# phlash/java-sdr

Hardware: AMD Instinct MI355X
Metric: IQ Msamples/s through FFT+FIR+BPSK demod, 2048-pt frames (higher is better)
Workload: dtype f64

## Files before the change

java-sdr_amd/csrc/fft_psd.hip:

```cpp
#include "fft_common.h"
#include <math.h>
#include <stdlib.h>
#include <vector>

namespace jsdr {

constexpr bool tw_direct(int P, int R) { return P * R <= 512; }
constexpr int tw_size(int P, int R) { return P <= 1 ? 0 : (tw_direct(P, R) ? 2 * P * (R - 1) : P); }
constexpr int tw_total(int R0, int R1, int R2, int R3)
{
    return tw_size(R0, R1) + (R2 > 1 ? tw_size(R0 * R1, R2) : 0) + (R3 > 1 ? tw_size(R0 * R1 * R2, R3) : 0);
}

constexpr int ilog2_c(int n) { return n <= 1 ? 0 : 1 + ilog2_c(n / 2); }

template <int R, int P>
__device__ __forceinline__ void apply_twiddles(float2 *v, int k, const float2 *tab)
{
    if constexpr (P > 1) {
        if constexpr (tw_direct(P, R)) {
#pragma unroll
            for (int r = 1; r < R; r++) {
                const float4 t = reinterpret_cast<const float4 *>(tab)[(r - 1) * P + k];
                v[r] = cmul2(v[r], make_float2(t.x, t.y), make_float2(t.z, t.w));
            }
        } else {
            float2 w1 = tab[k];
            float2 w[R], wq[R];
            w[1] = w1;
            wq[1] = cquad(w1);
#pragma unroll
            for (int r = 2; r < R; r++) {
                w[r] = (r & 1) ? cmul2(w[r - 1], w1, wq[1]) : cmul2(w[r / 2], w[r / 2], wq[r / 2]);
                wq[r] = cquad(w[r]);
            }
#pragma unroll
            for (int r = 1; r < R; r++) v[r] = cmul2(v[r], w[r], wq[r]);
        }
    }
}

template <int R, int... Rs>
__device__ __forceinline__ void store_lds(float2 *dst, const float2 *v, int j0, int p, std::integer_sequence<int, Rs...>)
{
    ((dst[lds_pad(j0 + Rs * p)] = v[cx_bitrev(Rs, R)]), ...);
}

template <int IN>
struct RawPoint {
    using type = int;
};
template <>
struct RawPoint<IN_F32> {
    using type = float2;
};
template <int N, int T, int IN, int R>
__device__ __forceinline__ void fft_fetch(const FftArgs &a, long long frame, int tid, typename RawPoint<IN>::type (&w)[R])
{
    constexpr int NB = N / R;
    static_assert(NB == T, "one first-pass butterfly per thread");
    const typename RawPoint<IN>::type *src = reinterpret_cast<const typename RawPoint<IN>::type *>(a.in) +
#ifdef JSDR_X_FFT_SMALLSET
        (frame & 8191) * N;
#else
        frame * N;
#endif
#pragma unroll
    for (int r = 0; r < R; r++) {
#ifdef JSDR_X_FFT_NOLOAD
        if constexpr (IN == IN_I16) w[r] = (tid + r * NB) * 2654435761u + (int)(size_t)src;
        else w[r] = make_float2((float)(tid + r), (float)(size_t)src);
#else
        w[r] = src[tid + r * NB];
#endif
    }
}

template <int N, int T, int IN, int OUT, int R, int P, bool FIRST, bool LAST, class RAW = int>
__device__ __forceinline__ void fft_pass(const FftArgs &a, long long frame, bool active, int tid, float2 *buf,
                                         const float2 *tab, Best &best, const RAW *raw = nullptr)
{
    constexpr int NB = N / R;
    static_assert(NB % T == 0, "butterflies per pass must be a multiple of the threads per frame");
    constexpr int ITERS = NB / T;
    constexpr int GROUP = LAST ? 1 : ITERS;
#pragma unroll
    for (int g0 = 0; g0 < ITERS; g0 += GROUP) {
        float2 v[GROUP][R];
#pragma unroll
        for (int gi = 0; gi < GROUP; gi++) {
            const int b = (g0 + gi) * T + tid;
            if constexpr (FIRST) {
                if (active) {
                    if constexpr (IN == IN_I16) {
                        const RAW *w = raw;
                        if ((a.ic | a.qc) == 0) {
#pragma unroll
                            for (int r = 0; r < R; r++)
                                v[gi][r] = make_float2(i16_to_float_java((int)(short)(w[r] & 0xffff)),
                                                       i16_to_float_java(w[r] >> 16));
                        } else {
#pragma unroll
                            for (int r = 0; r < R; r++) {
                                int si = java_short_add((int)(short)(w[r] & 0xffff), a.ic);
                                int sq = java_short_add(w[r] >> 16, a.qc);
                                v[gi][r] = make_float2(i16_to_float_java(si), i16_to_float_java(sq));
                            }
                        }
                    } else {
#pragma unroll
                        for (int r = 0; r < R; r++) v[gi][r] = raw[r];
                    }
                } else {
#pragma unroll
                    for (int r = 0; r < R; r++) v[gi][r] = make_float2(0.f, 0.f);
                }
            } else {
#pragma unroll
                for (int r = 0; r < R; r++) v[gi][r] = buf[lds_pad(b + r * NB)];
            }
            apply_twiddles<R, P>(v[gi], b & (P - 1), tab);
            dft_reg<R>(v[gi]);
        }
        if constexpr (!FIRST && !LAST) __syncthreads();
#pragma unroll
        for (int gi = 0; gi < GROUP; gi++) {
            const int b = (g0 + gi) * T + tid;
            const int k = b & (P - 1);
            const int j0 = (b - k) * R + k;
            if constexpr (!LAST) {
                store_lds<R>(buf, v[gi], j0, P, std::make_integer_sequence<int, R>{});
            } else if (active) {
                if constexpr (OUT == OUT_SPEC) {
                    float2 *dst = reinterpret_cast<float2 *>(a.out) + frame * N;
#pragma unroll
                    for (int r = 0; r < R; r++) dst[j0 + r * P] = v[gi][cx_bitrev(r, R)];
                } else {
                    constexpr float L2 = 3.0102999566398120f;
                    constexpr float OFF = 3.0102999566398120f * (2.0f - 2.0f * (float)ilog2_c(N));
                    float *dst = a.out + frame * (N + 2);
                    float db[R];
#pragma unroll
                    for (int r = 0; r < R; r++) {
                        float2 x = v[gi][cx_bitrev(r, R)];
                        db[r] = L2 * __log2f(x.x * x.x + x.y * x.y) + OFF;
#ifndef JSDR_X_FFT_NOSTORE
                        dst[j0 + r * P] = db[r];
#endif
                    }
                    float gm = db[0];
#pragma unroll
                    for (int r = 1; r < R; r++) gm = fmaxf(gm, db[r]);
                    int gk = 0x7fffffff;
#pragma unroll
                    for (int r = R - 1; r >= 0; r--) gk = (db[r] == gm) ? j0 + r * P : gk;
                    const bool take = (gm > best.v) | ((gm == best.v) & (gk < best.k));
                    best.v = take ? gm : best.v;
                    best.k = take ? gk : best.k;
                }
            }
        }
    }
    if constexpr (!LAST) __syncthreads();
}

template <int N, int T, int IN, int OUT, int R0, int R1, int R2, int R3>
__device__ __forceinline__ void fft_frame(const FftArgs &a, long long frame, long long next, int tid, float2 *buf,
                                          const float2 *tw_lds, float *red_val, int *red_idx, int frame_in_block,
                                          typename RawPoint<IN>::type (&raw)[R0])
{
    using RAW = typename RawPoint<IN>::type;
    constexpr bool active = true;
    constexpr int NPASS = (R1 == 1) ? 1 : (R2 == 1) ? 2 : (R3 == 1) ? 3 : 4;
    static_assert(NPASS >= 2, "the first pass must not be the last");
    static_assert(R0 * R1 * R2 * R3 == N, "radix plan must multiply to N");
    Best best;
    best.v = -3.402823466e+38f;
    best.k = 0x7fffffff;
    constexpr int O1 = 0, O2 = tw_size(R0, R1), O3 = O2 + tw_size(R0 * R1, R2);
    fft_pass<N, T, IN, OUT, R0, 1, true, false, RAW>(a, frame, active, tid, buf, tw_lds, best, raw);
    auto prefetch = [&] { fft_fetch<N, T, IN, R0>(a, next, tid, raw); };
    if constexpr (NPASS == 2) prefetch();
    fft_pass<N, T, IN, OUT, R1, R0, false, NPASS == 2>(a, frame, active, tid, buf, tw_lds + O1, best);
    if constexpr (NPASS >= 3) {
        if constexpr (NPASS == 3) prefetch();
        fft_pass<N, T, IN, OUT, R2, R0 * R1, false, NPASS == 3>(a, frame, active, tid, buf, tw_lds + O2, best);
    }
    if constexpr (NPASS >= 4) {
        prefetch();
        fft_pass<N, T, IN, OUT, R3, R0 * R1 * R2, false, NPASS == 4>(a, frame, active, tid, buf, tw_lds + O3, best);
    }

    if constexpr (OUT == OUT_PSD) {
        float bestv = best.v;
        int bestk = best.k;
        constexpr int W = (T < 64) ? T : 64;
#pragma unroll
        for (int off = W / 2; off >= 1; off >>= 1) {
            float ov = __shfl_xor(bestv, off, W);
            int ok = __shfl_xor(bestk, off, W);
            const bool take = (ov > bestv) | ((ov == bestv) & (ok < bestk));
            bestv = take ? ov : bestv;
            bestk = take ? ok : bestk;
        }
        if constexpr (T > 64) {
            constexpr int NW = T / 64;
            if ((tid & 63) == 0) {
                red_val[frame_in_block * NW + (tid >> 6)] = bestv;
                red_idx[frame_in_block * NW + (tid >> 6)] = bestk;
            }
            __syncthreads();
            if (tid == 0) {
                for (int w = 1; w < NW; w++) {
                    float ov = red_val[frame_in_block * NW + w];
                    int ok = red_idx[frame_in_block * NW + w];
                    if (ov > bestv || (ov == bestv && ok < bestk)) {
                        bestv = ov;
                        bestk = ok;
                    }
                }
            }
        }
        if (tid == 0 && active) {
            int p = (bestv > -3.402823466e+38f) ? 2 * bestk : -1;
            float m = (p >= 0) ? bestv : -3.402823466e+38f;
            const int datlen = 2 * N;
            if (p >= datlen / 2) p -= datlen;
            int hz = (int)((unsigned)p * (unsigned)a.rate) / datlen;
            float *dst = a.out + frame * (N + 2);
            dst[N] = (float)hz;
            dst[N + 1] = m;
        }
    }
}

template <int N, int T, int FPB, int IN, int OUT, int R0, int R1, int R2, int R3, bool TWG = false>
__global__ __launch_bounds__(T *FPB, (N == 2048 ? 4 : 1)) void k_fft(FftArgs a)
{
    extern __shared__ __align__(16) unsigned char smem[];
    constexpr int FE = lds_frame_elems(N);
    constexpr int TWN = TWG ? 0 : tw_total(R0, R1, R2, R3);
    float2 *tw_own = reinterpret_cast<float2 *>(smem);
    float2 *bufs = tw_own + TWN;
    float *red_val = reinterpret_cast<float *>(bufs + (size_t)FPB * FE);
    int *red_idx = reinterpret_cast<int *>(red_val + FPB * ((T + 63) / 64));
    const float2 *tw_lds = TWG ? a.tw : tw_own;

    const int tid_b = threadIdx.x;
    if constexpr (!TWG) {
        for (int i = tid_b; i < TWN; i += T * FPB) tw_own[i] = a.tw[i];
        __syncthreads();
    }

    const int fib = tid_b / T;
    const int tid = tid_b - fib * T;
    float2 *buf = bufs + (size_t)fib * FE;
    const long long ngroups = (a.nframes + FPB - 1) / FPB;
    auto frame_of = [&](long long g) {
        long long f = g * FPB + fib;
        return f < a.nframes ? f : a.nframes - 1;
    };
    typename RawPoint<IN>::type raw[R0];
    if ((long long)blockIdx.x < ngroups) fft_fetch<N, T, IN, R0>(a, frame_of(blockIdx.x), tid, raw);
    for (long long g = blockIdx.x; g < ngroups; g += gridDim.x) {
        const long long gn = g + gridDim.x;
        fft_frame<N, T, IN, OUT, R0, R1, R2, R3>(a, frame_of(g), frame_of(gn < ngroups ? gn : g), tid, buf, tw_lds, red_val,
                                                 red_idx, fib, raw);
        __syncthreads();
    }
}

template <int N, int FPB, int T, int R0, int R1, int R2, int R3, bool TWG = false>
constexpr size_t fft_lds_bytes()
{
    return sizeof(float2) * ((TWG ? (size_t)0 : (size_t)tw_total(R0, R1, R2, R3)) + (size_t)FPB * lds_frame_elems(N)) +
           (sizeof(float) + sizeof(int)) * FPB * ((T + 63) / 64);
}

struct Launcher {
    void (*launch)(const FftArgs &, int grid, hipStream_t) = nullptr;
    int frames_per_block = 0;
    size_t lds_bytes = 0;
    int block = 0;
    int radix[4] = {1, 1, 1, 1};
};

template <int N, int T, int FPB, int IN, int OUT, int R0, int R1, int R2, int R3, bool TWG = false>
static void launch_impl(const FftArgs &a, int grid, hipStream_t s)
{
    constexpr size_t lds = fft_lds_bytes<N, FPB, T, R0, R1, R2, R3, TWG>();
    hipLaunchKernelGGL((k_fft<N, T, FPB, IN, OUT, R0, R1, R2, R3, TWG>), dim3(grid), dim3(T * FPB), lds, s, a);
}

template <int N, int T, int FPB, int R0, int R1, int R2, int R3, bool TWG = false>
static Launcher make_launcher(int in, int out)
{
    Launcher l;
    l.frames_per_block = FPB;
    l.block = T * FPB;
    l.lds_bytes = fft_lds_bytes<N, FPB, T, R0, R1, R2, R3, TWG>();
    l.radix[0] = R0;
    l.radix[1] = R1;
    l.radix[2] = R2;
    l.radix[3] = R3;
    if (in == IN_I16 && out == OUT_PSD) l.launch = launch_impl<N, T, FPB, IN_I16, OUT_PSD, R0, R1, R2, R3, TWG>;
    if (in == IN_F32 && out == OUT_PSD) l.launch = launch_impl<N, T, FPB, IN_F32, OUT_PSD, R0, R1, R2, R3, TWG>;
    if (in == IN_F32 && out == OUT_SPEC) l.launch = launch_impl<N, T, FPB, IN_F32, OUT_SPEC, R0, R1, R2, R3, TWG>;
    return l;
}

static Launcher pick_launcher(int n, int in, int out)
{
    switch (n) {
        case 64: return make_launcher<64, 8, 32, 8, 8, 1, 1>(in, out);
        case 128: return make_launcher<128, 8, 32, 16, 8, 1, 1>(in, out);
        case 256: return make_launcher<256, 16, 16, 16, 16, 1, 1>(in, out);
        case 512: return make_launcher<512, 64, 4, 8, 8, 8, 1>(in, out);
        case 1024: return make_launcher<1024, 64, 4, 16, 8, 8, 1>(in, out);
        case 2048: return make_launcher<2048, 128, 2, 16, 16, 8, 1>(in, out);
        case 4096: return make_launcher<4096, 256, 1, 16, 16, 16, 1>(in, out);
        case 8192: return make_launcher<8192, 512, 1, 16, 16, 8, 4>(in, out);
        default: return Launcher();
    }
}

}

using namespace jsdr;

struct jsdr_fft {
    int n = 0;
    int rate = 0;
    DevBuf<float2> tw;
    DevBuf<unsigned char> in_stage;
    DevBuf<float> out_stage;
    PinnedStage pin;
    bool pin_lazy_done = false;
    int num_cu = 256;
    bool mixed = false;
    MixedPlan mplan;
    bool rt = false;
    bool direct = false;
    long long last_items = 0, last_grid = 0;
    int share_wgs_per_cu = 0;
};

static int fft_run(jsdr_fft *h, const void *in_dev, int in_kind, int out_kind, long long nframes, int ic, int qc,
                   float *out_dev, hipStream_t s)
{
    JSDR_REQUIRE(h, "fft: null handle");
    JSDR_REQUIRE(in_dev && out_dev, "fft: null buffer");
    JSDR_REQUIRE(nframes >= 0, "fft: negative frame count");
    if (nframes == 0) return JSDR_OK;
    FftArgs a;
    if (h->rt) {
        a.in = in_dev;
        a.out = out_dev;
        a.tw = h->tw.p;
        a.nframes = nframes;
        a.rate = h->rate;
        a.ic = ic;
        a.qc = qc;
        return rt_launch(a, h->n, in_kind, out_kind, h->num_cu, s);
    }
    if (h->direct) {
        a.in = in_dev;
        a.out = out_dev;
        a.tw = nullptr;
        a.nframes = nframes;
        a.rate = h->rate;
        a.ic = ic;
        a.qc = qc;
        return dft_any_launch(a, h->n, in_kind, out_kind, h->num_cu, s);
    }
    if (h->mixed) {
        a.in = in_dev;
        a.out = out_dev;
        a.tw = h->tw.p;
        a.nframes = nframes;
        a.rate = h->rate;
        a.ic = ic;
        a.qc = qc;
        if (h->mplan.split2)
            return mixed_launch_split2(h->mplan, a, in_kind, out_kind, h->num_cu, s);
        static const int mgrid = [] { const char *e = knob("JSDR_MIXED_GRID"); return e ? atoi(e) : 16; }();
        long long cap = (long long)h->num_cu * mgrid;
        return mixed_launch(h->mplan, a, in_kind, out_kind, (int)(nframes < cap ? nframes : cap), s);
    }
    Launcher l = pick_launcher(h->n, in_kind, out_kind);
    JSDR_REQUIRE(l.launch, "fft: no kernel for n=%d in=%d out=%d", h->n, in_kind, out_kind);
    a.in = in_dev;
    a.out = out_dev;
    a.tw = h->tw.p;
    a.nframes = nframes;
    a.rate = h->rate;
    a.ic = ic;
    a.qc = qc;
    long long groups = (nframes + l.frames_per_block - 1) / l.frames_per_block;
    long long per_cu = (long long)(160 * 1024 / l.lds_bytes);
    if (per_cu < 1) per_cu = 1;
    if (per_cu * l.block > 2048) per_cu = 2048 / l.block;
    static const int mult = [] {
        const char *e = knob("JSDR_FFT_GRID_MULT");
        const int v = e ? atoi(e) : 0;
        return v > 0 ? v : 4;
    }();
    long long cap = (long long)h->num_cu * per_cu * mult;
    static const int abs_grid = [] {
        const char *e = knob("JSDR_FFT_GRID_ABS");
        return e ? atoi(e) : 0;
    }();
    if (abs_grid > 0) cap = abs_grid;
    if (h->share_wgs_per_cu > 0) cap = (long long)h->num_cu * h->share_wgs_per_cu;
    int grid = (int)(groups < cap ? groups : cap);
    h->last_items = groups;
    h->last_grid = grid;
    l.launch(a, grid, s);
    JSDR_LAUNCH_CHECK();
    return JSDR_OK;
}

extern "C" {

int jsdr_fft_create(jsdr_fft **out, int n, int rate)
{
    JSDR_REQUIRE(out, "jsdr_fft_create: null handle pointer");
    *out = nullptr;
    MixedPlan mp;
    const bool pow2 = n >= 64 && n <= 8192 && (n & (n - 1)) == 0;
    const bool mixed = !pow2 && mixed_plan(n, mp);
    const bool rt = !pow2 && !mixed && rt_supported(n);
    const bool direct = !pow2 && !mixed && !rt && dft_any_supported(n);
    JSDR_REQUIRE(pow2 || mixed || rt || direct,
                 "jsdr_fft_create: n=%d unsupported (2 .. 20000 samples)", n);
    JSDR_REQUIRE(rate > 0, "jsdr_fft_create: rate must be positive");
    int dev = 0;
    JSDR_HIP_TRY(hipGetDevice(&dev));
    hipDeviceProp_t prop;
    JSDR_HIP_TRY(hipGetDeviceProperties(&prop, dev));
    jsdr_fft *h = new jsdr_fft();
    h->n = n;
    h->rate = rate;
    h->num_cu = prop.multiProcessorCount > 0 ? prop.multiProcessorCount : 256;
    if (direct) {
        h->direct = true;
        if (h->in_stage.alloc((size_t)n * 8) != JSDR_OK || h->out_stage.alloc((size_t)n + 2) != JSDR_OK) {
            jsdr_fft_destroy(h);
            return JSDR_ERR;
        }
        *out = h;
        return JSDR_OK;
    }
    if (rt) {
        h->rt = true;
        std::vector<float2> rtw;
        rt_twiddles(n, rtw);
        if (h->tw.alloc(rtw.size() ? rtw.size() : 1) != JSDR_OK || h->in_stage.alloc((size_t)n * 8) != JSDR_OK ||
            h->out_stage.alloc((size_t)n + 2) != JSDR_OK ||
            (rtw.size() && hipMemcpy(h->tw.p, rtw.data(), sizeof(float2) * rtw.size(), hipMemcpyHostToDevice) != hipSuccess)) {
            set_error("jsdr_fft_create: run-time-plan setup failed");
            jsdr_fft_destroy(h);
            return JSDR_ERR;
        }
        *out = h;
        return JSDR_OK;
    }
    if (mixed) {
        h->mixed = true;
        h->mplan = mp;
        std::vector<float2> mtw((size_t)mp.tw_count);
        mixed_twiddles(mp, mtw.data());
        if (h->tw.alloc(mtw.size()) != JSDR_OK || h->in_stage.alloc((size_t)n * 8) != JSDR_OK ||
            h->out_stage.alloc((size_t)n + 2) != JSDR_OK ||
            hipMemcpy(h->tw.p, mtw.data(), sizeof(float2) * mtw.size(), hipMemcpyHostToDevice) != hipSuccess) {
            set_error("jsdr_fft_create: mixed-radix setup failed");
            jsdr_fft_destroy(h);
            return JSDR_ERR;
        }
        *out = h;
        return JSDR_OK;
    }
    Launcher l = pick_launcher(n, IN_I16, OUT_PSD);
    std::vector<float2> tw;
    int P = l.radix[0];
    for (int pass = 1; pass < 4 && l.radix[pass] > 1; pass++) {
        const int R = l.radix[pass];
        const double base = -2.0 * 3.14159265358979323846 / ((double)P * (double)R);
        if (tw_direct(P, R)) {
            for (int r = 1; r < R; r++)
                for (int k = 0; k < P; k++) {
                    double ang = base * (double)k * (double)r;
                    const float2 w = make_float2((float)cos(ang), (float)sin(ang));
                    tw.push_back(w);
                    tw.push_back(make_float2(-w.y, w.x));
                }
        } else {
            for (int k = 0; k < P; k++) {
                double ang = base * (double)k;
                tw.push_back(make_float2((float)cos(ang), (float)sin(ang)));
            }
        }
        P *= R;
    }
    if ((int)tw.size() != tw_total(l.radix[0], l.radix[1], l.radix[2], l.radix[3])) {
        set_error("jsdr_fft_create: internal twiddle layout mismatch (%d)", (int)tw.size());
        delete h;
        return JSDR_ERR;
    }
    if (h->tw.alloc(tw.size()) != JSDR_OK || h->in_stage.alloc((size_t)n * 8) != JSDR_OK ||
        h->out_stage.alloc((size_t)n + 2) != JSDR_OK) {
        jsdr_fft_destroy(h);
        return JSDR_ERR;
    }
    if (hipMemcpy(h->tw.p, tw.data(), sizeof(float2) * tw.size(), hipMemcpyHostToDevice) != hipSuccess) {
        set_error("jsdr_fft_create: twiddle upload failed");
        jsdr_fft_destroy(h);
        return JSDR_ERR;
    }
    *out = h;
    return JSDR_OK;
}

int jsdr_fft_destroy(jsdr_fft *h)
{
    if (!h) return JSDR_OK;
    h->tw.release();
    h->in_stage.release();
    h->out_stage.release();
    h->pin.release();
    delete h;
    return JSDR_OK;
}

int jsdr_fft_batch_f32(jsdr_fft *h, const float *iq_dev, int64_t nframes, float *psd_dev, void *stream)
{
    return fft_run(h, iq_dev, IN_F32, OUT_PSD, nframes, 0, 0, psd_dev, as_stream(stream));
}

int jsdr_fft_set_cu_share(jsdr_fft *h, int wgs_per_cu)
{
    JSDR_REQUIRE(h && wgs_per_cu >= 0 && wgs_per_cu <= 16, "jsdr_fft_set_cu_share: bad argument");
    h->share_wgs_per_cu = wgs_per_cu;
    return JSDR_OK;
}

const char *jsdr_fft_kernel(jsdr_fft *h)
{
    if (!h) return "";
    return h->rt ? "k_fft_rt" : h->direct ? "k_dft_any" : h->mixed ? (h->mplan.split2 ? "k_fft_mixed_dual" : "k_fft_mixed") : "k_fft";
}

int jsdr_fft_last_launch(jsdr_fft *h, int64_t *work_items, int64_t *workgroups)
{
    JSDR_REQUIRE(h && work_items && workgroups, "jsdr_fft_last_launch: null argument");
    *work_items = h->last_items;
    *workgroups = h->last_grid;
    return JSDR_OK;
}

int jsdr_fft_batch_i16(jsdr_fft *h, const int16_t *raw_dev, int64_t nframes, int ic, int qc, float *psd_dev,
                       void *stream)
{
    return fft_run(h, raw_dev, IN_I16, OUT_PSD, nframes, ic, qc, psd_dev, as_stream(stream));
}

int jsdr_fft_spectrum_f32(jsdr_fft *h, const float *iq_dev, int64_t nframes, float *spec_dev, void *stream)
{
    return fft_run(h, iq_dev, IN_F32, OUT_SPEC, nframes, 0, 0, spec_dev, as_stream(stream));
}

static int fft_receive(jsdr_fft *h, const void *in_host, size_t in_bytes, int in_kind, int ic, int qc, float *psd_host)
{
    const size_t out_bytes = sizeof(float) * ((size_t)h->n + 2), in_room = (size_t)h->n * 8;
    if (h->pin.p && h->pin.bytes >= in_room + out_bytes) {
        memcpy(h->pin.p, in_host, in_bytes);
        SyncOnExit guard;
        JSDR_HIP_TRY(hipMemcpyAsync(h->in_stage.p, h->pin.p, in_bytes, hipMemcpyHostToDevice, 0));
        if (fft_run(h, h->in_stage.p, in_kind, OUT_PSD, 1, ic, qc, h->out_stage.p, 0) != JSDR_OK) return JSDR_ERR;
        JSDR_HIP_TRY(hipMemcpyAsync(h->pin.p + in_room, h->out_stage.p, out_bytes, hipMemcpyDeviceToHost, 0));
        JSDR_HIP_TRY(hipStreamSynchronize(0));
        guard.armed = false;
        memcpy(psd_host, h->pin.p + in_room, out_bytes);
        return JSDR_OK;
    }
    JSDR_HIP_TRY(hipMemcpy(h->in_stage.p, in_host, in_bytes, hipMemcpyHostToDevice));
    if (fft_run(h, h->in_stage.p, in_kind, OUT_PSD, 1, ic, qc, h->out_stage.p, 0) != JSDR_OK) return JSDR_ERR;
    JSDR_HIP_TRY(hipMemcpy(psd_host, h->out_stage.p, out_bytes, hipMemcpyDeviceToHost));
    return JSDR_OK;
}

int jsdr_fft_receive_f32(jsdr_fft *h, const float *iq_host, float *psd_host)
{
    JSDR_REQUIRE(h && iq_host && psd_host, "jsdr_fft_receive_f32: null argument");
    if (!h->pin_lazy_done && !h->pin.p) {
        h->pin.alloc((size_t)h->n * 8 + sizeof(float) * ((size_t)h->n + 2));
        h->pin_lazy_done = true;
    }
    return fft_receive(h, iq_host, sizeof(float) * 2 * (size_t)h->n, IN_F32, 0, 0, psd_host);
}

int jsdr_fft_receive_i16(jsdr_fft *h, const int16_t *raw_host, int ic, int qc, float *psd_host)
{
    JSDR_REQUIRE(h && raw_host && psd_host, "jsdr_fft_receive_i16: null argument");
    if (!h->pin_lazy_done && !h->pin.p) {
        h->pin.alloc((size_t)h->n * 8 + sizeof(float) * ((size_t)h->n + 2));
        h->pin_lazy_done = true;
    }
    return fft_receive(h, raw_host, sizeof(int16_t) * 2 * (size_t)h->n, IN_I16, ic, qc, psd_host);
}

}
```

Before: 240,900.

## Stage 2048-point PSD rows in LDS and store them with wide coalesced writes

For the 2048-point int16-to-PSD kernel, the last FFT pass now writes dB values into a linear LDS image instead of scattering scalar stores to global memory. After the reduction the row is copied out as coalesced float2 stores (float4 stores and wide int4 loads are optional variants). The aim is to replace strided scalar global writes with contiguous wide ones. The cost is an extra LDS round trip and barrier in the last pass, plus a runtime alignment check with a fallback to the narrow kernel.

```diff
diff --git a/java-sdr_amd/csrc/fft_psd.hip b/java-sdr_amd/csrc/fft_psd.hip
--- a/java-sdr_amd/csrc/fft_psd.hip
+++ b/java-sdr_amd/csrc/fft_psd.hip
@@ -54,11 +54,30 @@
 struct RawPoint<IN_F32> {
     using type = float2;
 };
-template <int N, int T, int IN, int R>
+enum { WIO_ST = 1, WIO_LD = 2, WIO_ST4 = 4 };
+
+template <int N, int T, int IN, int R, int WIO = 0>
 __device__ __forceinline__ void fft_fetch(const FftArgs &a, long long frame, int tid, typename RawPoint<IN>::type (&w)[R])
 {
     constexpr int NB = N / R;
     static_assert(NB == T, "one first-pass butterfly per thread");
+    if constexpr ((WIO & WIO_LD) != 0) {
+        static_assert(IN == IN_I16 && R % 4 == 0, "wide loads: int16 input, whole 16-byte groups");
+        const int4 *src4 = reinterpret_cast<const int4 *>(a.in) + frame * (N / 4);
+#pragma unroll
+        for (int q = 0; q < R / 4; q++) {
+#ifdef JSDR_X_FFT_NOLOAD
+            const int4 t = make_int4((tid + q) * 2654435761u + (int)(size_t)src4, tid, q, tid ^ q);
+#else
+            const int4 t = src4[tid + q * T];
+#endif
+            w[4 * q] = t.x;
+            w[4 * q + 1] = t.y;
+            w[4 * q + 2] = t.z;
+            w[4 * q + 3] = t.w;
+        }
+        return;
+    }
     const typename RawPoint<IN>::type *src = reinterpret_cast<const typename RawPoint<IN>::type *>(a.in) +
 #ifdef JSDR_X_FFT_SMALLSET
         (frame & 8191) * N;
@@ -76,14 +95,28 @@
     }
 }
 
-template <int N, int T, int IN, int OUT, int R, int P, bool FIRST, bool LAST, class RAW = int>
+template <int T, int R>
+__device__ __forceinline__ void fft_deal(int (&w)[R], float *lin, int tid)
+{
+    int4 *l4 = reinterpret_cast<int4 *>(lin);
+#pragma unroll
+    for (int q = 0; q < R / 4; q++) l4[tid + q * T] = make_int4(w[4 * q], w[4 * q + 1], w[4 * q + 2], w[4 * q + 3]);
+    __syncthreads();
+    const int *l1 = reinterpret_cast<const int *>(lin);
+#pragma unroll
+    for (int r = 0; r < R; r++) w[r] = l1[tid + r * T];
+    __syncthreads();
+}
+
+template <int N, int T, int IN, int OUT, int R, int P, bool FIRST, bool LAST, class RAW = int, bool LIN = false>
 __device__ __forceinline__ void fft_pass(const FftArgs &a, long long frame, bool active, int tid, float2 *buf,
-                                         const float2 *tab, Best &best, const RAW *raw = nullptr)
-{
+                                         const float2 *tab, Best &best, const RAW *raw = nullptr, float *lin = nullptr)
+{
+    static_assert(!LIN || (LAST && OUT == OUT_PSD), "the linear image takes PSD rows");
     constexpr int NB = N / R;
     static_assert(NB % T == 0, "butterflies per pass must be a multiple of the threads per frame");
     constexpr int ITERS = NB / T;
-    constexpr int GROUP = LAST ? 1 : ITERS;
+    constexpr int GROUP = (LAST && !LIN) ? 1 : ITERS;
 #pragma unroll
     for (int g0 = 0; g0 < ITERS; g0 += GROUP) {
         float2 v[GROUP][R];
@@ -122,7 +155,7 @@
             apply_twiddles<R, P>(v[gi], b & (P - 1), tab);
             dft_reg<R>(v[gi]);
         }
-        if constexpr (!FIRST && !LAST) __syncthreads();
+        if constexpr (!FIRST && (!LAST || LIN)) __syncthreads();
 #pragma unroll
         for (int gi = 0; gi < GROUP; gi++) {
             const int b = (g0 + gi) * T + tid;
@@ -144,8 +177,9 @@
                     for (int r = 0; r < R; r++) {
                         float2 x = v[gi][cx_bitrev(r, R)];
                         db[r] = L2 * __log2f(x.x * x.x + x.y * x.y) + OFF;
+                        if constexpr (LIN) lin[j0 + r * P] = db[r];
 #ifndef JSDR_X_FFT_NOSTORE
-                        dst[j0 + r * P] = db[r];
+                        else dst[j0 + r * P] = db[r];
 #endif
                     }
                     float gm = db[0];
@@ -164,12 +198,17 @@
     if constexpr (!LAST) __syncthreads();
 }
 
-template <int N, int T, int IN, int OUT, int R0, int R1, int R2, int R3>
+template <int N, int T, int IN, int OUT, int R0, int R1, int R2, int R3, int WIO = 0>
 __device__ __forceinline__ void fft_frame(const FftArgs &a, long long frame, long long next, int tid, float2 *buf,
                                           const float2 *tw_lds, float *red_val, int *red_idx, int frame_in_block,
-                                          typename RawPoint<IN>::type (&raw)[R0])
+                                          typename RawPoint<IN>::type (&raw)[R0], float *lin = nullptr)
 {
     using RAW = typename RawPoint<IN>::type;
+    constexpr bool WST = (WIO & (WIO_ST | WIO_ST4)) != 0;
+    static_assert(WIO == 0 || (IN == IN_I16 && OUT == OUT_PSD && T > 64), "wide I/O: the int16 -> PSD kernel");
+    int shift = 0;
+    if constexpr ((WIO & WIO_ST4) != 0) shift = (int)((reinterpret_cast<size_t>(a.out + frame * (N + 2)) >> 2) & 3);
+    if constexpr ((WIO & WIO_LD) != 0) fft_deal<T, R0>(raw, lin, tid);
     constexpr bool active = true;
     constexpr int NPASS = (R1 == 1) ? 1 : (R2 == 1) ? 2 : (R3 == 1) ? 3 : 4;
     static_assert(NPASS >= 2, "the first pass must not be the last");
@@ -179,16 +218,19 @@
     best.k = 0x7fffffff;
     constexpr int O1 = 0, O2 = tw_size(R0, R1), O3 = O2 + tw_size(R0 * R1, R2);
     fft_pass<N, T, IN, OUT, R0, 1, true, false, RAW>(a, frame, active, tid, buf, tw_lds, best, raw);
-    auto prefetch = [&] { fft_fetch<N, T, IN, R0>(a, next, tid, raw); };
+    auto prefetch = [&] { fft_fetch<N, T, IN, R0, WIO>(a, next, tid, raw); };
     if constexpr (NPASS == 2) prefetch();
-    fft_pass<N, T, IN, OUT, R1, R0, false, NPASS == 2>(a, frame, active, tid, buf, tw_lds + O1, best);
+    fft_pass<N, T, IN, OUT, R1, R0, false, NPASS == 2, int, WST && NPASS == 2>(a, frame, active, tid, buf, tw_lds + O1, best,
+                                                                               nullptr, lin + shift);
     if constexpr (NPASS >= 3) {
         if constexpr (NPASS == 3) prefetch();
-        fft_pass<N, T, IN, OUT, R2, R0 * R1, false, NPASS == 3>(a, frame, active, tid, buf, tw_lds + O2, best);
+        fft_pass<N, T, IN, OUT, R2, R0 * R1, false, NPASS == 3, int, WST && NPASS == 3>(a, frame, active, tid, buf, tw_lds + O2,
+                                                                                        best, nullptr, lin + shift);
     }
     if constexpr (NPASS >= 4) {
         prefetch();
-        fft_pass<N, T, IN, OUT, R3, R0 * R1 * R2, false, NPASS == 4>(a, frame, active, tid, buf, tw_lds + O3, best);
+        fft_pass<N, T, IN, OUT, R3, R0 * R1 * R2, false, NPASS == 4, int, WST>(a, frame, active, tid, buf, tw_lds + O3, best,
+                                                                               nullptr, lin + shift);
     }
 
     if constexpr (OUT == OUT_PSD) {
@@ -210,6 +252,26 @@
                 red_idx[frame_in_block * NW + (tid >> 6)] = bestk;
             }
             __syncthreads();
+#ifndef JSDR_X_FFT_NOSTORE
+            if constexpr ((WIO & WIO_ST4) != 0) {
+                float *dst = a.out + frame * (N + 2);
+                const float4 *l4 = reinterpret_cast<const float4 *>(lin);
+                float4 *g4 = reinterpret_cast<float4 *>(dst - shift);
+#pragma unroll
+                for (int q = 0; q < N / (4 * T); q++) {
+                    const float4 t = l4[tid + q * T];
+                    if (q == 0 && shift != 0 && tid == 0) *reinterpret_cast<float2 *>(dst) = make_float2(t.z, t.w);
+                    else g4[tid + q * T] = t;
+                }
+                if (shift != 0 && tid == T - 1)
+                    *reinterpret_cast<float2 *>(dst + N - 2) = *reinterpret_cast<const float2 *>(lin + N);
+            } else if constexpr ((WIO & WIO_ST) != 0) {
+                float2 *g2 = reinterpret_cast<float2 *>(a.out + frame * (N + 2));
+                const float2 *l2 = reinterpret_cast<const float2 *>(lin);
+#pragma unroll
+                for (int q = 0; q < N / (2 * T); q++) g2[tid + q * T] = l2[tid + q * T];
+            }
+#endif
             if (tid == 0) {
                 for (int w = 1; w < NW; w++) {
                     float ov = red_val[frame_in_block * NW + w];
@@ -234,7 +296,7 @@
     }
 }
 
-template <int N, int T, int FPB, int IN, int OUT, int R0, int R1, int R2, int R3, bool TWG = false>
+template <int N, int T, int FPB, int IN, int OUT, int R0, int R1, int R2, int R3, bool TWG = false, int WIO = 0>
 __global__ __launch_bounds__(T *FPB, (N == 2048 ? 4 : 1)) void k_fft(FftArgs a)
 {
     extern __shared__ __align__(16) unsigned char smem[];
@@ -255,17 +317,19 @@
     const int fib = tid_b / T;
     const int tid = tid_b - fib * T;
     float2 *buf = bufs + (size_t)fib * FE;
+    static_assert(WIO == 0 || 2 * FE >= N + 6, "a linear row must fit the frame's image");
+    float *lin = reinterpret_cast<float *>(buf + ((TWN + fib * FE) & 1));
     const long long ngroups = (a.nframes + FPB - 1) / FPB;
     auto frame_of = [&](long long g) {
         long long f = g * FPB + fib;
         return f < a.nframes ? f : a.nframes - 1;
     };
     typename RawPoint<IN>::type raw[R0];
-    if ((long long)blockIdx.x < ngroups) fft_fetch<N, T, IN, R0>(a, frame_of(blockIdx.x), tid, raw);
+    if ((long long)blockIdx.x < ngroups) fft_fetch<N, T, IN, R0, WIO>(a, frame_of(blockIdx.x), tid, raw);
     for (long long g = blockIdx.x; g < ngroups; g += gridDim.x) {
         const long long gn = g + gridDim.x;
-        fft_frame<N, T, IN, OUT, R0, R1, R2, R3>(a, frame_of(g), frame_of(gn < ngroups ? gn : g), tid, buf, tw_lds, red_val,
-                                                 red_idx, fib, raw);
+        fft_frame<N, T, IN, OUT, R0, R1, R2, R3, WIO>(a, frame_of(g), frame_of(gn < ngroups ? gn : g), tid, buf, tw_lds,
+                                                      red_val, red_idx, fib, raw, lin);
         __syncthreads();
     }
 }
@@ -279,17 +343,29 @@
 
 struct Launcher {
     void (*launch)(const FftArgs &, int grid, hipStream_t) = nullptr;
+    void (*launch_wide)(const FftArgs &, int grid, hipStream_t) = nullptr;
     int frames_per_block = 0;
     size_t lds_bytes = 0;
     int block = 0;
     int radix[4] = {1, 1, 1, 1};
 };
 
-template <int N, int T, int FPB, int IN, int OUT, int R0, int R1, int R2, int R3, bool TWG = false>
+template <int N, int T, int FPB, int IN, int OUT, int R0, int R1, int R2, int R3, bool TWG = false, int WIO = 0>
 static void launch_impl(const FftArgs &a, int grid, hipStream_t s)
 {
     constexpr size_t lds = fft_lds_bytes<N, FPB, T, R0, R1, R2, R3, TWG>();
-    hipLaunchKernelGGL((k_fft<N, T, FPB, IN, OUT, R0, R1, R2, R3, TWG>), dim3(grid), dim3(T * FPB), lds, s, a);
+    hipLaunchKernelGGL((k_fft<N, T, FPB, IN, OUT, R0, R1, R2, R3, TWG, WIO>), dim3(grid), dim3(T * FPB), lds, s, a);
+}
+
+#ifndef JSDR_X_FFT_WIO
+#define JSDR_X_FFT_WIO (WIO_ST)
+#endif
+static bool fft_wide_ok(const void *in, const float *out)
+{
+    static const bool narrow = [] { const char *e = knob("JSDR_FFT_NARROW"); return e && atoi(e) != 0; }();
+    if (narrow) return false;
+    if (((JSDR_X_FFT_WIO) & WIO_LD) != 0 && (reinterpret_cast<size_t>(in) & 15) != 0) return false;
+    return (reinterpret_cast<size_t>(out) & 7) == 0;
 }
 
 template <int N, int T, int FPB, int R0, int R1, int R2, int R3, bool TWG = false>
@@ -317,7 +393,12 @@
         case 256: return make_launcher<256, 16, 16, 16, 16, 1, 1>(in, out);
         case 512: return make_launcher<512, 64, 4, 8, 8, 8, 1>(in, out);
         case 1024: return make_launcher<1024, 64, 4, 16, 8, 8, 1>(in, out);
-        case 2048: return make_launcher<2048, 128, 2, 16, 16, 8, 1>(in, out);
+        case 2048: {
+            Launcher l = make_launcher<2048, 128, 2, 16, 16, 8, 1>(in, out);
+            if (in == IN_I16 && out == OUT_PSD)
+                l.launch_wide = launch_impl<2048, 128, 2, IN_I16, OUT_PSD, 16, 16, 8, 1, false, (JSDR_X_FFT_WIO)>;
+            return l;
+        }
         case 4096: return make_launcher<4096, 256, 1, 16, 16, 16, 1>(in, out);
         case 8192: return make_launcher<8192, 512, 1, 16, 16, 8, 4>(in, out);
         default: return Launcher();
@@ -415,7 +496,8 @@
     int grid = (int)(groups < cap ? groups : cap);
     h->last_items = groups;
     h->last_grid = grid;
-    l.launch(a, grid, s);
+    if (l.launch_wide && fft_wide_ok(in_dev, out_dev)) l.launch_wide(a, grid, s);
+    else l.launch(a, grid, s);
     JSDR_LAUNCH_CHECK();
     return JSDR_OK;
 }
```

New measurement: 236,200, median of 2. 0.98x the previous value.
